# hasindu2008/sigtk

Hardware: AMD Instinct MI355X
Metric: event_raw_samples_per_sec (higher is better)
Workload: dtype f32+f64; 1 GPU; sigtk event (DNA params) on 10000 synthetic reads x 100000 samples per GPU (BASELINE configs[1]), device-resident; reads_per_gpu=10000, samples_per_read=100000, samples_per_gpu=1000000000, fallback_reads=0, rerun_chunks=0, long_detector_replays=66844, long_detector_replay_indices=87529, split_reads=0, batches_in_flight=1, parallelism=reads sharded across ranks, no collective

## Files before the change

### sigtk_amd/build.py

```python
from __future__ import annotations

import os
import shutil
import subprocess
import sys

PKG = os.path.dirname(os.path.abspath(__file__))
ROOT = os.path.dirname(PKG)
CSRC = os.path.join(PKG, "csrc")
HOST = os.path.join(PKG, "host")
LIB = os.path.join(PKG, "libsigtk_gpu.so")
CLI = os.path.join(PKG, "sigtk-amd")
CLI_ASAN = os.path.join(PKG, "sigtk-amd-asan")

EVENT_SOURCES = ["event_launch.hip", "event_whole.hip", "event_seg.hip", "event_multi.hip", "event_fallback.hip"]
HIP_SOURCES = ["api.hip", "api_stat.hip", *EVENT_SOURCES, "stat_launch.hip", "stat_lane.hip", "stat_wave.hip", "stat_long.hip",
               "misc_kernels.hip", "svb_kernels.hip", "sigtext_kernels.hip", "inflate_kernels.hip", "deflate_kernels.hip", "zstd_kernels.hip", "zrec_kernels.hip", "ent_kernels.hip",
               "qts_kernels.hip", "text_kernels.hip", "slow5_text_kernels.hip", "sref_kernels.hip", "ss_kernels.hip", "job.hip", "shims.hip"]
SOURCE_FLAGS = {"event_whole.hip": ["-fno-slp-vectorize"], "event_multi.hip": ["-fno-slp-vectorize"]}
HIPCC_FLAGS = ["--offload-arch=gfx950", "-O3", "-std=c++17", "-ffp-contract=off",
               "-fhip-fp32-correctly-rounded-divide-sqrt", "-fPIC", "-shared", "-Wall",
               "-Wno-unused-function", "-Wno-bitwise-instead-of-logical", "-Wno-c++20-extensions", "-Wno-pass-failed"]


# ... 36 lines not shown
    if jobs:
        with ThreadPoolExecutor(max_workers=min(len(jobs), max(1, (os.cpu_count() or 2) - 1))) as ex:
            list(ex.map(run, jobs))
    if force or jobs or not _newer(LIB, objs):
        run([cc, "--offload-arch=gfx950", "-shared", "-fPIC", "-o", LIB, *objs])
    return LIB


def build_variant(tag: str, defines, sources=(*EVENT_SOURCES, "api.hip"), verbose: bool = False) -> str:
    build_lib(verbose=verbose)
    vdir = os.path.join(PKG, "_variants")
    os.makedirs(vdir, exist_ok=True)
    cc = hipcc()
    flags = [f for f in HIPCC_FLAGS if f != "-shared"] + list(defines)
    objs = []
    for s_ in HIP_SOURCES:
        base = s_[:-4]
        if s_ in sources:
            obj = os.path.join(vdir, "%s_%s.o" % (base, tag))
            cmd = [cc, *flags, *SOURCE_FLAGS.get(s_, []), "-c", "-o", obj, os.path.join(CSRC, s_)]
            if verbose:
                print(" ".join(cmd), file=sys.stderr)
            subprocess.check_call(cmd)
        else:
            obj = os.path.join(PKG, "build", base + ".o")
        objs.append(obj)
    out = os.path.join(vdir, "libsigtk_gpu_%s.so" % tag)
    subprocess.check_call([cc, "--offload-arch=gfx950", "-shared", "-fPIC", "-o", out, *objs])
    return out


def build_cli(force: bool = False, verbose: bool = False) -> str:
    if not os.path.isdir(HOST):
        return ""
    srcs = sorted(os.path.join(HOST, f) for f in os.listdir(HOST) if f.endswith(".c"))
    if not srcs:
        return ""
    deps = srcs + [os.path.join(HOST, f) for f in os.listdir(HOST) if f.endswith(".h")]
    deps.append(os.path.join(ROOT, "include", "sigtk_gpu.h"))
    deps.append(os.path.join(CSRC, "text_format.h"))
    if not force and _newer(CLI, deps) and _newer(CLI, [LIB]):
        return CLI
    cmd = ["gcc", "-O2", "-std=c99", "-D_GNU_SOURCE", "-Wall", "-I", os.path.join(ROOT, "include"), "-o", CLI, *srcs,
           "-L", PKG, "-lsigtk_gpu", "-Wl,-rpath,$ORIGIN", "-Wl,-rpath,/opt/rocm/lib", "-lz", "-lm", "-lpthread"]
    if verbose:
        print(" ".join(cmd), file=sys.stderr)
    subprocess.check_call(cmd)
    return CLI


def build_cli_asan(force: bool = False, verbose: bool = False) -> str:
    srcs = sorted(os.path.join(HOST, f) for f in os.listdir(HOST) if f.endswith(".c"))
    deps = srcs + [os.path.join(HOST, f) for f in os.listdir(HOST) if f.endswith(".h")]
    deps.append(os.path.join(ROOT, "include", "sigtk_gpu.h"))
    deps.append(os.path.join(CSRC, "text_format.h"))
    if not os.path.exists(LIB):
        build_lib(verbose=verbose)
    if not force and _newer(CLI_ASAN, deps) and _newer(CLI_ASAN, [LIB]):
        return CLI_ASAN
    cmd = ["gcc", "-O1", "-g", "-fno-omit-frame-pointer", "-fsanitize=address,undefined", "-fno-sanitize-recover=undefined",
           "-std=c99", "-D_GNU_SOURCE", "-Wall", "-I", os.path.join(ROOT, "include"), "-o", CLI_ASAN, *srcs,
           "-L", PKG, "-lsigtk_gpu", "-Wl,-rpath,$ORIGIN", "-Wl,-rpath,/opt/rocm/lib", "-lz", "-lm", "-lpthread"]
    if verbose:
        print(" ".join(cmd), file=sys.stderr)
    subprocess.check_call(cmd)
    return CLI_ASAN


def build_tools(force: bool = False, verbose: bool = False) -> None:
    tdir = os.path.join(ROOT, "tools")
    math_h = os.path.join(CSRC, "tstat_math.h")
    numerics = ["-ffp-contract=off", "-fhip-fp32-correctly-rounded-divide-sqrt"]
    for name in ("rsq_check", "valu_rate", "fetch_calib", "sqrt_cert_gpu"):
        src = os.path.join(tdir, name + ".hip")
        exe = os.path.join(tdir, name)
        deps = [src] + ([os.path.join(tdir, "valu_rate_tests.inc")] if name == "valu_rate" else [])
        deps += [math_h] if name == "sqrt_cert_gpu" else []
        if not os.path.exists(src) or (not force and _newer(exe, deps)):
            continue
        cmd = [hipcc(), "--offload-arch=gfx950", "-O2", *(numerics if name == "sqrt_cert_gpu" else []), "-o", exe, src]
        if verbose:
            print(" ".join(cmd), file=sys.stderr)
        subprocess.check_call(cmd)
    src, exe = os.path.join(tdir, "sqrt_check.cpp"), os.path.join(tdir, "sqrt_check")
    if os.path.exists(src) and (force or not _newer(exe, [src, math_h])):
        cmd = ["g++", "-O2", "-std=c++17", "-ffp-contract=off", "-pthread", "-o", exe, src]
        if verbose:
            print(" ".join(cmd), file=sys.stderr)
        subprocess.check_call(cmd)


if __name__ == "__main__":
    if "--variant" in sys.argv:
        i = sys.argv.index("--variant")
        print(build_variant(sys.argv[i + 1], [x for x in sys.argv[i + 2:] if x.startswith("-D")], verbose=True))
        sys.exit(0)
    build_tools(force="--force" in sys.argv, verbose=True)
    build_lib(force="--force" in sys.argv, verbose=True)
    build_cli(force="--force" in sys.argv, verbose=True)
    if "--asan" in sys.argv:
        build_cli_asan(force="--force" in sys.argv, verbose=True)
```

### sigtk_amd/csrc/event_detect.h

```cpp
#pragma once
#include <utility>

#include "event_device.h"

namespace sgk {

template <int W1>
struct LzCfg {
    static constexpr int W2 = 2 * W1;
    static constexpr int R = 16;
    static constexpr int NP = (W1 == 3) ? 8 : 16;
    static constexpr int NA = (W1 == 3) ? 4 : 8;
    static constexpr int NL = (W1 == 3) ? 8 : 16;
    static constexpr int H1 = W1 / 2;
};
static_assert(LzCfg<3>::NP >= 8 && LzCfg<7>::NP >= 16, "prefix ring holds P(i) .. P(i+W2+1)");

constexpr int LZ_NONE = -(1 << 29);
constexpr int LZ_NREC = 8;
constexpr int LZ_RING_WORDS = 16;

struct LzSnap {
    LzSnapState init[64];
    LzSnapState at_e[64];
    LzSnapState st0[64];
};
__device__ inline bool lz_equal(const LzSnapState &a, const LzSnapState &b) {
    return a.sp == b.sp && __float_as_int(a.sv) == __float_as_int(b.sv) && a.lm == b.lm && a.r0 == b.r0 &&
           a.bits == b.bits;
}
struct LzLds {
    uint32_t ring[64][LZ_RING_WORDS + 1];
    LzSnap snap;
    LzRun runs[64][LZ_NREC];
    int nrec[64];
};

template <typename T>
__device__ __attribute__((noinline)) float tstat_exact_at(const T *base, Scale sc, int i, int w) {
    double A = 0.0, A2 = 0.0, B = 0.0, B2 = 0.0;
    for (int k = 0; k < w; ++k) {
        const float xa = to_pa(base[i - w + k], sc);
        const float xb = to_pa(base[i + k], sc);
        A = A + (double)xa;
        A2 = A2 + (double)(xa * xa);
        B = B + (double)xb;
        B2 = B2 + (double)(xb * xb);
    }
    if (w == 3) return sgk_tstat_ref<3>(A, A2, B, B2);
    if (w == 6) return sgk_tstat_ref<6>(A, A2, B, B2);
    if (w == 7) return sgk_tstat_ref<7>(A, A2, B, B2);
    return sgk_tstat_ref<14>(A, A2, B, B2);
}

template <typename T>
struct Lead16;
template <>
struct Lead16<int16_t> {
    uint32_t w[8];
    template <int U>
    __device__ __forceinline__ float get(const Scale &sc) const {
        const int v = (U & 1) ? ((int)w[U / 2] >> 16) : (int)(short)(w[U / 2] & 0xffffu);
        const float shifted = (float)v + sc.offf;
        return shifted * sc.unit;
    }
};
template <>
struct Lead16<float> {
    float w[16];
    template <int U>
    __device__ __forceinline__ float get(const Scale &) const { return w[U]; }
};
typedef uint32_t sgk_u32x4_a4 __attribute__((ext_vector_type(4), aligned(4)));

template <typename T>
__device__ __attribute__((noinline)) Lead16<T> lead_fix_head(Lead16<T> g, int pos, T first) {
    T tmp[16];
    __builtin_memcpy(tmp, g.w, sizeof(tmp));
#pragma unroll
    for (int k = 0; k < 16; ++k) tmp[k] = (pos + k < 0) ? first : tmp[k];
    __builtin_memcpy(g.w, tmp, sizeof(tmp));
    return g;
}

constexpr int REP_MAX_EVENTS = 32;
struct RepairCtx {
    const double *P, *P2;
    const int *ev;
    int nev;
    bool all_dirty;
};

__device__ __attribute__((noinline)) float tstat_prefix_at(const double *P, const double *P2, int i, int w) {
    const double p0 = P[i], q0 = P2[i];
    const double A = p0 - P[i - w], A2 = q0 - P2[i - w], B = P[i + w] - p0, B2 = P2[i + w] - q0;
    if (w == 3) return sgk_tstat_ref<3>(A, A2, B, B2);
    if (w == 6) return sgk_tstat_ref<6>(A, A2, B, B2);
    if (w == 7) return sgk_tstat_ref<7>(A, A2, B, B2);
    return sgk_tstat_ref<14>(A, A2, B, B2);
}

template <int W1>
__device__ __forceinline__ void repair_mark(const RepairCtx &rep, int &next_t, int q0, unsigned cnt1, unsigned cnt2,
                                            unsigned &bad1, unsigned &bad2) {
    constexpr int W2 = 2 * W1;
    if (rep.all_dirty) {
#pragma unroll
        for (int u = 0; u < 4; ++u) {
            if ((unsigned)(q0 + u - W1) < cnt1) bad1 |= 1u << u;
            if ((unsigned)(q0 + u - W2) < cnt2) bad2 |= 1u << u;
        }
        return;
    }
    if (next_t > q0 + 3 + W2 - 1) return;
    int nt = 0x7fffffff;
    for (int k = 0; k < rep.nev; ++k) {
        const int t = rep.ev[k];
#pragma unroll
        for (int u = 0; u < 4; ++u) {
            const int i = q0 + u;
            if ((unsigned)(i - t + W1 - 1) < (unsigned)(2 * W1) && (unsigned)(i - W1) < cnt1) bad1 |= 1u << u;
            if ((unsigned)(i - t + W2 - 1) < (unsigned)(2 * W2) && (unsigned)(i - W2) < cnt2) bad2 |= 1u << u;
        }
        if (t + W2 >= q0 + 4 && t < nt) nt = t;
    }
    next_t = nt;
}

constexpr int LZ_PRE = LZ_RING_WORDS;
__device__ __attribute__((noinline)) void lz_emit_slow(uint32_t *ring, unsigned long long *bm, int flushed,
                                                       int i_begin, int s, int e, int p, int cur) {
    const int own_lo = s - i_begin;
    if (p < own_lo) {
        if (cur >= own_lo) ring[LZ_PRE] = (uint32_t)(i_begin + p);
        return;
    }
    if (p >= flushed) {
        atomicOr(&ring[(p >> 5) & (LZ_RING_WORDS - 1)], 1u << (p & 31));
    } else {
        const int pa = i_begin + p;
        if (pa >= s && pa < e) atomicOr(reinterpret_cast<uint32_t *>(bm) + (pa >> 5), 1u << (pa & 31));
    }
}
__device__ __attribute__((noinline)) int lz_record(LzRun *runs, int nrec, int a, int b, int s, int e, int n) {
    if ((b >= s && b < e) || (b == n && e == n && s < n)) {
        if (nrec < LZ_NREC) {
            runs[nrec].a = a;
            runs[nrec].b = b;
        }
        ++nrec;
    }
    return nrec;
}

struct Redo4 {
    float v[4];
};
template <int W1, typename T, bool FLAGGED>
__device__ __attribute__((noinline)) Redo4 redo_quad(const T *base, Scale sc, const double *P, const double *P2, int i0,
                                                     unsigned cnt1, unsigned bits, float t0, float t1, float t2,
                                                     float t3) {
    Redo4 r;
    r.v[0] = t0; r.v[1] = t1; r.v[2] = t2; r.v[3] = t3;
#pragma unroll
    for (int k = 0; k < 4; ++k) {
        if ((bits >> k) & 1u) {
            const int i = i0 + k;
            float v = 0.0f;
            if ((unsigned)(i - W1) < cnt1) {
                if constexpr (FLAGGED) v = tstat_prefix_at(P, P2, i, W1);
                else v = tstat_exact_at<T>(base, sc, i, W1);
            }
            r.v[k] = v;
        }
    }
    return r;
}

typedef unsigned long long lmask_t;
__device__ __forceinline__ bool lane_of(lmask_t m) { return __builtin_amdgcn_inverse_ballot_w64(m); }

template <int W1, typename T, bool FLAGGED>
struct LazyPass {
    using C = LzCfg<W1>;
    static constexpr int W2 = C::W2, R = C::R, NP = C::NP, NA = C::NA, NL = C::NL, H1 = C::H1;
    double Ps[NP], Pq[NP];
    SgkARole ar[NA];
    SgkLSide ls[NL];
    float t1[4];
    lmask_t nk[4];
    lmask_t hc[4];
    Lead16<T> cur;
    float sv;
    int sp;
    lmask_t inpk, val, strong;
    lmask_t hist[H1 + 1];
    uint32_t bw;
    int lm, r0;
    lmask_t hot;
    int nrec;
    uint32_t *ring;
    LzRun *runs;
    const T *base;
    int lo, hi;
    Scale sc;
    int n, s, e, i_begin, ib, jb, flushed;
    unsigned cnt1, cnt2;
    lmask_t done;
    bool slow;
    bool oldpeak;
    unsigned long long *bm;
    RepairCtx rep;
    int next_t;
    int dirty;

    __device__ __forceinline__ void load_lead(Lead16<T> &dst, int pos) const {
        int p = pos > hi - 16 ? hi - 16 : pos;
        p = p < lo ? lo : p;
        constexpr int NV = 16 * (int)sizeof(T) / 16;
        const sgk_u32x4_a4 *src = reinterpret_cast<const sgk_u32x4_a4 *>(base + p);
        sgk_u32x4_a4 v[NV];
#pragma unroll
        for (int k = 0; k < NV; ++k) v[k] = src[k];
        __builtin_memcpy(dst.w, v, sizeof(dst.w));
        if (pos < 0) dst = lead_fix_head<T>(dst, pos, base[0]);
    }

    template <int U>
    __device__ __forceinline__ void tstep() {
        const float xn = cur.template get<U>(sc);
        const float xqn = xn * xn;
        Ps[(U + W2 + 1) % NP] = Ps[(U + W2) % NP] + (double)xn;
        Pq[(U + W2 + 1) % NP] = Pq[(U + W2) % NP] + (double)xqn;
        const double p0 = Ps[U % NP], q0 = Pq[U % NP];
        const double b1 = Ps[(U + W1) % NP] - p0, b1q = Pq[(U + W1) % NP] - q0;
        const double b2 = Ps[(U + W2) % NP] - p0, b2q = Pq[(U + W2) % NP] - q0;
        const SgkLSide lb = sgk_lside<W2>(b2, b2q);
        if constexpr (!FLAGGED) {
            bool cv_ok, tail_ok;
            t1[U & 3] = sgk_tstat_try_ab<W1>(b1, b1q, ar[(U + NA - W1) % NA], cv_ok, tail_ok);
            nk[U & 3] = ~(__ballot(cv_ok) & __ballot(tail_ok));
            ar[U % NA] = sgk_arole<W1, true>(b1, b1q);
            hc[U & 3] = ~__ballot(sgk_long_cold<W2>(ls[(U + NL - W2) % NL], lb));
            ls[U % NL] = lb;
        } else {
            bool ok;
            const float v = sgk_tstat_try_ab<W1>(b1, b1q, ar[(U + NA - W1) % NA], ok);
            ok = ok && sgk_try_domain<W1>(b1, b1q, ar[(U + NA - W1) % NA]);
            const double a_s = Ps[(U + W2) % NP], b_s = (double)xn, r_s = Ps[(U + W2 + 1) % NP];
            const double a_q = Pq[(U + W2) % NP], b_q = (double)xqn, r_q = Pq[(U + W2 + 1) % NP];
            const double t_s = r_s - a_s, t_q = r_q - a_q;
            const double e_s = (a_s - (r_s - t_s)) + (b_s - t_s), e_q = (a_q - (r_q - t_q)) + (b_q - t_q);
            const bool clean = U > dirty;
            if (e_s != 0.0 || e_q != 0.0) dirty = dirty > U + 2 * W2 ? dirty : U + 2 * W2;
            ok = ok && clean;
            ar[U % NA] = sgk_arole<W1, false>(b1, b1q);
            bool cold = sgk_long_cold<W2>(ls[(U + NL - W2) % NL], lb);
            cold = cold && clean && sgk_lside_domain(ls[(U + NL - W2) % NL]) && sgk_lside_domain(lb);
            ls[U % NL] = lb;
            t1[U & 3] = v;
            nk[U & 3] = ~__ballot(ok);
            hc[U & 3] = ~__ballot(cold);
        }
    }

    template <bool SLOW>
    __device__ __forceinline__ void dstep_core(const int u, const float v, const lmask_t hck, const lmask_t live) {
        constexpr float ph = DetParam<W1>::ph, thr1 = DetParam<W1>::thr1;
        const float d1 = v - sv;
        const float ee = lane_of(inpk) ? d1 : -d1;
        lmask_t P = __ballot(ee > 0.0f);
        lmask_t Q = __ballot(ee < -ph);
        const lmask_t Tt = __ballot(v > thr1);
        if constexpr (SLOW) {
            P &= live;
            Q &= live;
        }
        const lmask_t ent = Q & ~inpk;
        const lmask_t pos = (inpk & P) | ent;
        strong = (pos & Tt) | (strong & ~pos);
        lmask_t dom = inpk & strong;
        if constexpr (SLOW) dom &= live;
        val = inpk & (val | (Q & strong));
        lmask_t recent = hist[0];
#pragma unroll
        for (int k = 1; k < H1; ++k) recent |= hist[k];
        lmask_t em = val & ~P & ~recent;
        if constexpr (SLOW) em &= live;
        const lmask_t upd = P | ent | em;
        const uint32_t bit = 1u << ((jb + u - H1 - 1) & 31);
        if (SLOW && oldpeak) {
            if (lane_of(em)) {
                lz_emit_slow(ring, bm, flushed, i_begin, s, e, jb + sp, jb + u);
                lm = sp;
                r0 = u;
            }
        } else {
            if (lane_of(em)) {
                bw |= bit;
                lm = sp;
                r0 = u;
            }
            const lmask_t erare = em & ~hist[H1];
            if (erare != 0ull) {
                if (lane_of(erare)) {
                    bw &= ~bit;
                    const int p = jb + sp, own = s - i_begin;
                    if (p >= own) atomicOr(&ring[(p >> 5) & (LZ_RING_WORDS - 1)], 1u << (p & 31));
                    else if (jb >= own) ring[LZ_PRE] = (uint32_t)(i_begin + p);
                }
            }
        }
        sv = lane_of(upd) ? v : sv;
        sp = lane_of(pos) ? u : sp;
        inpk = (inpk & ~em) | ent;
        val = val & ~em;
// ... 30 lines not shown
    __device__ __forceinline__ void dstep_edge() {
        if constexpr (U == H1 + 1) {
            if ((jb & 16) == 0) bw_advance();
        }
        const lmask_t live = ~done & __ballot((unsigned)(ib + U) < (unsigned)n);
        dstep_core<true>(U, t1[U & 3], hc[U & 3], live);
    }
    __device__ __forceinline__ void slow_fix(const int u0) {
#pragma unroll
        for (int k = 0; k < 4; ++k) {
            const bool in1 = (unsigned)(ib + u0 + k - W1) < cnt1;
            t1[k] = in1 ? t1[k] : 0.0f;
            nk[k] &= __ballot(in1);
            hc[k] &= __ballot((unsigned)(ib + u0 + k - W2) < cnt2);
        }
    }

    template <int U0>
    __device__ __forceinline__ void quad() {
        tstep<U0>();
        tstep<U0 + 1>();
        tstep<U0 + 2>();
        tstep<U0 + 3>();
        if (slow) slow_fix(U0);
        if constexpr (FLAGGED) {
            unsigned bad1 = 0u, bad2 = 0u;
            repair_mark<W1>(rep, next_t, ib + U0, cnt1, cnt2, bad1, bad2);
#pragma unroll
            for (int k = 0; k < 4; ++k) {
                nk[k] |= __ballot(((bad1 >> k) & 1u) != 0u);
                hc[k] |= __ballot(((bad2 >> k) & 1u) != 0u);
            }
        }
        const lmask_t anybad = (nk[0] | nk[1] | nk[2] | nk[3]) & ~done;
        if (anybad != 0ull) {
            if (lane_of(anybad)) {
                const unsigned bits = (lane_of(nk[0]) ? 1u : 0u) | (lane_of(nk[1]) ? 2u : 0u) |
                                      (lane_of(nk[2]) ? 4u : 0u) | (lane_of(nk[3]) ? 8u : 0u);
                const Redo4 r4 = redo_quad<W1, T, FLAGGED>(base, sc, rep.P, rep.P2, ib + U0, cnt1, bits, t1[0], t1[1],
                                                           t1[2], t1[3]);
                t1[0] = r4.v[0]; t1[1] = r4.v[1]; t1[2] = r4.v[2]; t1[3] = r4.v[3];
            }
        }
        if (slow) {
            dstep_edge<U0>();
            dstep_edge<U0 + 1>();
            dstep_edge<U0 + 2>();
            dstep_edge<U0 + 3>();
        } else {
            dstep<U0>();
            dstep<U0 + 1>();
            dstep<U0 + 2>();
            dstep<U0 + 3>();
        }
    }

    template <int K>
    __device__ __forceinline__ void init_step(double &ps, double &pq, const float (&w)[2 * W2], double (&hs)[W2 + 1],
                                              double (&hq)[W2 + 1]) {
        const float x = w[K];
        ps = ps + (double)x;
        pq = pq + (double)(x * x);
        constexpr int k1 = K + 1;
        if constexpr (k1 <= W2) { hs[k1] = ps; hq[k1] = pq; }
        if constexpr (k1 >= W2) { Ps[(k1 - W2) % NP] = ps; Pq[(k1 - W2) % NP] = pq; }
        if constexpr (k1 >= W2 && k1 < W2 + W1) {
            constexpr int pr = k1 - W1;
            ar[((k1 - W1 - W2) % NA + NA) % NA] = sgk_arole<W1, !FLAGGED>(ps - hs[pr], pq - hq[pr]);
        }
        if constexpr (k1 >= W2 && k1 < 2 * W2) {
            constexpr int pr = k1 - W2;
            ls[((k1 - 2 * W2) % NL + NL) % NL] = sgk_lside<W2>(ps - hs[pr], pq - hq[pr]);
        }
    }
    template <int... Ks>
    __device__ __forceinline__ void init_rings(const float (&w)[2 * W2], std::integer_sequence<int, Ks...>) {
        double ps = 0.0, pq = 0.0;
        double hs[W2 + 1], hq[W2 + 1];
        hs[0] = 0.0;
        hq[0] = 0.0;
        (init_step<Ks>(ps, pq, w, hs, hq), ...);
    }

    template <int... Qs>
    __device__ __forceinline__ void block(std::integer_sequence<int, Qs...>) {
        (quad<4 * Qs>(), ...);
    }
};

__device__ __forceinline__ void lz_flush(uint32_t *ring, unsigned long long *bm, int i_begin, int p0, int own_lo,
                                         int own_hi) {
    uint16_t *bm16 = reinterpret_cast<uint16_t *>(bm);
#pragma unroll
    for (int k = 0; k < 8; ++k) {
        const int p = p0 + 32 * k;
        const int wi = (p >> 5) & (LZ_RING_WORDS - 1);
        const uint32_t w = ring[wi];
        ring[wi] = 0u;
        if (p >= own_lo && p < own_hi) bm16[(i_begin + p) >> 4] = (uint16_t)(w & 0xffffu);
        if (p + 16 >= own_lo && p + 16 < own_hi) bm16[(i_begin + p + 16) >> 4] = (uint16_t)(w >> 16);
    }
}

template <int W1, typename T, bool FLAGGED>
__device__ __forceinline__ void pass_lazy(const ReadCtx<T> &rc, bool given, int lead, int steps, bool active, int s,
                                          int e, LzLds *L, const RepairCtx *rep, bool by_progress = false) {
    using LP = LazyPass<W1, T, FLAGGED>;
    constexpr int W2 = LP::W2, R = LP::R;
    if (!__any(active)) return;
    const int l = lane_id();
    LP f;
    f.n = (int)rc.n;
    f.s = active ? s : 0x7fffffff;
    f.e = active ? e : 0x7fffffff;
    f.bm = rc.bm;
    f.sc = rc.sc;
    f.base = rc.base;
    f.lo = (int)(rc.lo < -(1 << 30) ? -(1 << 30) : rc.lo);
    f.hi = (int)(rc.hi > 0x7fffffffLL ? 0x7fffffffLL : rc.hi);
    f.ring = L->ring[l];
    f.runs = L->runs[l];
    const int n = f.n;
    const int i_begin = s - lead;
    f.i_begin = i_begin;
#pragma unroll
    for (int k = 0; k < LZ_RING_WORDS; ++k) f.ring[k] = 0u;
    if (active) f.ring[LZ_PRE] = 0xffffffffu;
#pragma unroll
    for (int k = 0; k < 4; ++k) { f.t1[k] = 0.0f; f.nk[k] = 0ull; f.hc[k] = 0ull; }
    {
        float w[2 * W2];
#pragma unroll
        for (int k = 0; k < 2 * W2; ++k) {
            int p = i_begin - W2 + k;
            p = p > f.hi - 1 ? f.hi - 1 : p;
            p = p < 0 ? 0 : p;
            w[k] = to_pa(f.base[p], f.sc);
        }
#pragma unroll
        for (int k = 0; k < LP::NP; ++k) { f.Ps[k] = 0.0; f.Pq[k] = 0.0; }
        f.init_rings(w, std::make_integer_sequence<int, 2 * W2>{});
        if (i_begin == 0) {
#pragma unroll
            for (int k = 0; k < LP::NA; ++k) f.ar[k].va = __builtin_nan("");
        }
    }
    f.load_lead(f.cur, i_begin + W2);

    f.sv = FLT_MAX;
    f.sp = 0;
    f.inpk = 0ull; f.val = 0ull; f.strong = 0ull; f.hot = 0ull;
#pragma unroll
    for (int k = 0; k <= LP::H1; ++k) f.hist[k] = 0ull;
    f.bw = 0u;
    f.lm = LZ_NONE;
    f.r0 = 0;
    if (__any(given)) {
        LzSnapState st = L->snap.st0[l];
        if (!given) { st.sp = -1; st.sv = FLT_MAX; st.lm = LZ_NONE; st.r0 = i_begin; st.bits = 0u; }
        f.sv = st.sv;
        f.inpk = __ballot((st.bits & 1u) != 0u);
        f.val = __ballot((st.bits & 2u) != 0u);
        f.strong = __ballot((st.bits & 4u) != 0u);
        f.hot = __ballot((st.bits & 8u) != 0u);
        f.sp = (st.bits & 1u) ? st.sp - i_begin : 0;
        f.lm = st.lm == LZ_NONE ? LZ_NONE : st.lm - W1 - i_begin;
#pragma unroll
        for (int k = 0; k <= LP::H1; ++k) f.hist[k] = __ballot((st.bits & 1u) && st.sp == i_begin - 1 - k);
        f.r0 = st.r0 - i_begin;
    }
    f.nrec = 0;
    f.done = ~__ballot(active);
    f.flushed = 0;
    if constexpr (FLAGGED) {
        f.dirty = 2 * W2;
        f.rep = *rep;
        f.next_t = 0x7fffffff;
        for (int k = 0; k < f.rep.nev; ++k) {
            const int t = f.rep.ev[k];
            if (t + W2 >= i_begin && t < f.next_t) f.next_t = t;
        }
    }
    const int main_steps = steps;
    f.cnt1 = (n - 2 * W1 + 1) > 0 ? (unsigned)(n - 2 * W1 + 1) : 0u;
    f.cnt2 = (n - 2 * W2 + 1) > 0 ? (unsigned)(n - 2 * W2 + 1) : 0u;
    const int own_lo = lead, own_hi = active ? lead + (e - s) : lead;

    auto snapshot = [&](int ib) -> LzSnapState {
        LzSnapState st;
        const bool ip = lane_of(f.inpk);
        st.sv = f.sv;
        st.sp = ip ? ib + f.sp : -1;
        st.lm = (f.lm + W1 < 0) ? LZ_NONE : ib + f.lm + W1;
        st.r0 = ib + max(f.r0, f.lm + W1 + 1);
        st.bits = (ip ? 1u : 0u) | ((ip && lane_of(f.val)) ? 2u : 0u) | ((ip && lane_of(f.strong)) ? 4u : 0u) |
                  (lane_of(f.hot) ? 8u : 0u);
        return st;
    };

    constexpr int PRIO_STEPS = 400;
    const int q1 = by_progress ? main_steps - 3 * PRIO_STEPS : -1, q2 = by_progress ? main_steps - 2 * PRIO_STEPS : -1,
              q3 = by_progress ? main_steps - PRIO_STEPS : -1;
    if (by_progress) {
        if (q1 > 0) __builtin_amdgcn_s_setprio(3);
        else if (q2 > 0) __builtin_amdgcn_s_setprio(2);
        else if (q3 > 0) __builtin_amdgcn_s_setprio(1);
        else __builtin_amdgcn_s_setprio(0);
    }
    int jb = 0;
    for (;;) {
        const int ib = i_begin + jb;
        if ((jb & 255) == 0 && jb >= 512) {
            lz_flush(f.ring, f.bm, i_begin, jb - 512, own_lo, own_hi);
            f.flushed = jb - 256;
        }
        const bool lane_edge = ib + R - 1 > n - W2;
        const lmask_t old_peak = __ballot(f.sp < -(256 - 2 * R)) | (__ballot(f.sp + jb < own_lo) & __ballot(jb == own_lo));
        f.oldpeak = (old_peak & f.inpk & ~f.done) != 0ull;
        f.slow = f.oldpeak || (__ballot(lane_edge) & ~f.done) != 0ull;
        f.ib = ib;
        f.jb = jb;
        Lead16<T> nxt;
        f.load_lead(nxt, ib + R + W2);
        f.block(std::make_integer_sequence<int, R / 4>{});
        f.cur = nxt;
        f.sp -= R;
        f.lm = f.lm < LZ_NONE ? LZ_NONE : f.lm - R;
// ... 6 lines not shown
        {
            const int nb = i_begin + jb;
            if (active && lead > 0 && jb == lead) L->snap.init[l] = snapshot(nb);
            if (active && nb == e) L->snap.at_e[l] = snapshot(nb);
            const lmask_t reach = __ballot(nb >= e) & ~f.done;
            if ((reach & f.hot) != 0ull) {
                if (lane_of(reach & f.hot) && e == n) f.nrec = lz_record(f.runs, f.nrec, nb + max(f.r0, f.lm + W1 + 1), n, s, e, n);
            }
            f.done |= reach;
            f.inpk &= ~reach;
            f.val &= ~reach;
            f.strong &= ~reach;
        }
        if (jb >= main_steps && f.done == ~0ull) break;
    }
    {
        const int p = jb - LP::H1 - 2 < 0 ? 0 : jb - LP::H1 - 2;
        atomicOr(&f.ring[(p >> 5) & (LZ_RING_WORDS - 1)], f.bw);
    }
    for (int p0 = f.flushed; p0 < jb; p0 += 256) lz_flush(f.ring, f.bm, i_begin, p0, own_lo, own_hi);
    if (active) L->nrec[l] = f.nrec;
}

template <int W1, typename T, bool FLAGGED, bool COLLECT = false>
__device__ inline void replay_run(const ReadCtx<T> &rc, const RepairCtx *rep, bool has, int i, int b, int bits_lo,
                           int bits_hi, EvHeader *hdr, int *found = nullptr) {
    if (has && b > i) atomicAdd(&hdr->n_replay_idx, (unsigned long long)(b - i));
    constexpr int W2 = 2 * W1;
    constexpr float ph = DetParam<W1>::ph, thr2 = DetParam<W1>::thr2;
    const int n = (int)rc.n;
    const unsigned cnt2 = (n - 2 * W2 + 1) > 0 ? (unsigned)(n - 2 * W2 + 1) : 0u;
    uint32_t *bm32 = reinterpret_cast<uint32_t *>(rc.bm);
    int lp = -1;
    float lv = FLT_MAX;
    bool lvalid = false;
    while (__any(has && i < b)) {
        if (has && i < b) {
            float v2 = 0.0f;
            if ((unsigned)(i - W2) < cnt2) {
                if constexpr (FLAGGED) v2 = tstat_prefix_at(rep->P, rep->P2, i, W2);
                else v2 = tstat_exact_at<T>(rc.base, rc.sc, i, W2);
            }
            if (lp < 0) {
                if (v2 < lv) {
                    lv = v2;
                } else if (v2 - lv > ph) {
                    lv = v2;
                    lp = i;
                }
            } else {
                if (v2 > lv) {
                    lv = v2;
                    lp = i;
                }
                if (lv - v2 > ph && lv > thr2) lvalid = true;
                if (lvalid && (i - lp) > W2 / 2) {
                    if (lp > 0 && lp < n && lp >= bits_lo && lp < bits_hi) {
                        if constexpr (COLLECT) *found = 1;
                        else atomicOr(&bm32[lp >> 5], 1u << (lp & 31));
                    }
                    lp = -1;
                    lv = v2;
                    lvalid = false;
                }
            }
            ++i;
        }
    }
}
template <int W1, typename T, bool FLAGGED>
__device__ void replay_long_runs(const ReadCtx<T> &rc, LzLds *L, const RepairCtx *rep, bool active, int bits_lo,
                                 EvHeader *hdr) {
    const int l = lane_id();
    const int nrec = active ? L->nrec[l] : 0;
    for (int k = 0; k < LZ_NREC; ++k) {
        const bool has = k < nrec;
        if (!__any(has)) break;
        const int i = has ? L->runs[l][k].a : 0;
        const int b = has ? L->runs[l][k].b : 0;
        replay_run<W1, T, FLAGGED>(rc, rep, has, i, b, bits_lo, 0x7fffffff, hdr);
    }
}

template <int W1, typename T, bool FLAGGED, bool MULTI = false>
__device__ __forceinline__ int detect_span(const ReadCtx<T> &rc, EvHeader *hdr, LzLds *L, const RepairCtx *rep,
                                           const int a, const int b, const int mode, const int lead_override,
                                           SegState *seg, const int lanes = 64) {
    const int n = (int)rc.n;
    if constexpr (!MULTI) {
        if (b <= a) return 0;
    }
    const int len = b - a;
    int lead = len < 32768 ? LEAD_DNA_SHORT : LEAD_DNA;
    if (W1 == 7) lead = len <= 32768 ? LEAD_RNA_SHORT : LEAD_RNA;
    if constexpr (MULTI) {
        const long long len64 = (long long)len * (64 / lanes);
        lead = len64 < 32768 ? LEAD_DNA_SHORT : LEAD_DNA;
        if (W1 == 7) lead = len64 <= 32768 ? LEAD_RNA_SHORT : LEAD_RNA;
    }
    if (lead_override > 0) lead = lead_override;
    const bool no_fast = (reinterpret_cast<uintptr_t>(rc.base) & 3u) != 0 || rc.hi < (int64_t)n + 16;
    if constexpr (!MULTI) {
        if (no_fast) return 1;
    }
    const int c = MULTI ? (lane_id() & (lanes - 1)) : lane_id();
    int K, s, e0, lead_c;
    if (mode == 1) {
        K = 16 * ((len + 1023) / 1024);
        s = a + c * K;
        e0 = s + K;
        lead_c = lead;
    } else {
        K = MULTI ? chunk_len_lanes(len, lead, lanes) : chunk_len_fast(len, lead);
        s = c == 0 ? a : a + c * K + lead;
        e0 = c == 0 ? a + lead + K : s + K;
        lead_c = c > 0 ? lead : 0;
    }
    int TT = lead + K;
    int Kmax = K;
    if constexpr (MULTI) {
#pragma unroll
        for (int d = 32; d >= 1; d >>= 1) {
            const int o = __shfl_xor(Kmax, d, 64), t = __shfl_xor(TT, d, 64);
            Kmax = o > Kmax ? o : Kmax;
            TT = t > TT ? t : TT;
        }
    }
    const int e = e0 < b ? e0 : b;
    const bool active = s < b && !(MULTI && no_fast);
    {
        LzSnapState z;
        z.sp = -1; z.sv = FLT_MAX; z.lm = LZ_NONE; z.r0 = 0; z.bits = 0u;
        L->snap.init[lane_id()] = z;
        L->snap.at_e[lane_id()] = z;
        L->nrec[lane_id()] = 0;
        L->ring[lane_id()][LZ_PRE] = 0xffffffffu;
    }
    bool run = active;
    bool first = true;
    const int l = lane_id();
    const uint32_t pol = FLAGGED ? 0u : prio_policy(rc.dev);
    for (int iter = 0; iter < 66; ++iter) {
        pass_lazy<W1, T, FLAGGED>(rc, first ? (mode == 2 && c == 0) : true, first ? lead_c : 0, first ? TT : Kmax, run, s, e,
                                  L, rep, first && (pol == 1u || pol == 2u));
        __syncthreads();
        const LzSnapState pe = L->snap.at_e[c > 0 ? l - 1 : l];
        const LzSnapState mine = L->snap.init[l];
        const bool bad = active && c > 0 && !lz_equal(pe, mine);
        const unsigned long long badmask = __ballot(bad);
        if (badmask == 0ull) break;
        __syncthreads();
        if (bad) {
            L->snap.init[l] = pe;
            L->snap.st0[l] = pe;
        }
        run = bad;
        first = false;
        if (l == 0) atomicAdd(&hdr->n_rerun, (uint32_t)__popcll(badmask));
        __syncthreads();
    }
    int rcode = 0;
    if constexpr (MULTI) {
        const unsigned long long over = __ballot(active && L->nrec[l] > LZ_NREC);
        const unsigned long long grp = (lanes >= 64 ? ~0ull : ((1ull << lanes) - 1ull)) << (l & ~(lanes - 1));
        if (no_fast) rcode = 1;
        else if (over & grp) rcode = 2;
    } else {
        if (__any(active && L->nrec[l] > LZ_NREC)) return 2;
    }
    const bool mine_ok = active && rcode == 0;
    if (seg) {
        const int last = __popcll(__ballot(active)) - 1;
        if (l == 0) {
            seg->init0 = L->snap.init[0];
            seg->end = L->snap.at_e[last];
        }
        const int nrec = active ? L->nrec[l] : 0;
        int ncross = 0;
        for (int k = 0; k < nrec; ++k) ncross += (L->runs[l][k].a < a) ? 1 : 0;
        const int incl = wave_incl_scan_i(ncross);
        const int total = wave_last_i(incl);
        if (total > SEG_CROSS_MAX) rcode = 2;
        else {
            int at = incl - ncross;
            for (int k = 0; k < nrec; ++k) {
                if (L->runs[l][k].a < a) seg->cross[at++] = L->runs[l][k];
            }
        }
        if (l == 0) seg->n_cross = total > SEG_CROSS_MAX ? 0u : (uint32_t)total;
    }
    const int pre = mine_ok ? (int)L->ring[l][LZ_PRE] : -1;
    const bool pre_out = pre >= 0 && pre < a;
    if (seg) {
        const int npre = pre_out ? 1 : 0;
        const int incl = wave_incl_scan_i(npre);
        const int total = wave_last_i(incl);
        if (total > SEG_PRE_MAX) rcode = 2;
        else if (npre) seg->pre[incl - 1] = pre;
        if (l == 0) seg->n_pre = total > SEG_PRE_MAX ? 0u : (uint32_t)total;
    }
    const unsigned long long hotm = __ballot(mine_ok && L->nrec[l] > 0);
    const bool anypre = __any(pre >= 0);
    if (hotm != 0ull || anypre) {
        if (l == 0 && hotm != 0ull) atomicAdd(&hdr->n_hot_runs, (uint32_t)__popcll(hotm));
        __threadfence_block();
        __syncthreads();
        if (pre >= 0 && !pre_out) atomicOr(reinterpret_cast<uint32_t *>(rc.bm) + (pre >> 5), 1u << (pre & 31));
        if (hotm != 0ull) replay_long_runs<W1, T, FLAGGED>(rc, L, rep, mine_ok, a, hdr);
    }
    return rcode;
}
template <int W1, typename T, bool FLAGGED>
__device__ __forceinline__ int detect_read_lazy(const ReadCtx<T> &rc, EvHeader *hdr, LzLds *L, const RepairCtx *rep) {
    const int n = (int)rc.n;
    if (n <= 0) return 0;
    return detect_span<W1, T, FLAGGED>(rc, hdr, L, rep, 0, n, 0, 0, nullptr);
}

}
```

### sigtk_amd/csrc/event_multi.hip

```cpp
#include "event_build.h"

namespace sgk {

template <int W1, typename T>
__global__ __launch_bounds__(64, (W1 == 3 ? DET_WAVES_DNA : DET_WAVES_RNA)) void k_event_multi(EvArgs a) {
    __shared__ EventLds L;
    const int lanes = (int)a.multi_lanes, G = 64 / lanes;
    const int l = lane_id();
    const uint32_t first = a.order ? a.order[a.n_reads + len_bucket(a.multi_max)] : 0u;
    const uint32_t nshort = a.n_reads - first;
    const uint32_t w0 = blockIdx.x * (uint32_t)G;
    if (w0 >= nshort) return;
    const uint32_t gi = (uint32_t)l / (uint32_t)lanes;
    const bool has = w0 + gi < nshort;
    const uint32_t idx = first + (has ? w0 + gi : w0);
    const uint32_t r = a.order ? a.order[idx] : idx;
    ReadCtx<T> rc = make_ctx<T>(a, r);
    const bool mine = has && !(a.max_segs && rc.n >= (int64_t)a.long_min);
    if (!mine) rc.n = 0;
    const int rcode = detect_span<W1, T, false, true>(rc, a.hdr, &L.lz, nullptr, 0, (int)rc.n, 0, a.lead_override, nullptr,
                                                      lanes);
    __builtin_amdgcn_fence(__ATOMIC_RELEASE, "workgroup");
    __syncthreads();
    __builtin_amdgcn_fence(__ATOMIC_ACQUIRE, "workgroup");
    for (int g = 0; g < G; ++g) {
        if (w0 + (uint32_t)g >= nshort) break;
        const uint32_t rg = (uint32_t)__builtin_amdgcn_readlane((int)r, g * lanes);
        const int code = __builtin_amdgcn_readlane(rcode, g * lanes);
        if (!__builtin_amdgcn_readlane((int)mine, g * lanes)) continue;
        const ReadCtx<T> rcg = make_ctx<T>(a, rg);
        build_read<T>(a, rcg, rg, &L.b, code != 0);
        __syncthreads();
    }
}

int launch_k_event_multi(int rna, bool float_input, hipStream_t st, const EvArgs &a) {
    const uint32_t per_wave = 64u / a.multi_lanes;
    const uint32_t grid = (a.n_reads + per_wave - 1) / per_wave;
    if (rna && float_input) SGK_LAUNCH("k_event_multi", (k_event_multi<7, float>), grid, 64, st, a);
    else if (rna) SGK_LAUNCH("k_event_multi", (k_event_multi<7, int16_t>), grid, 64, st, a);
    else if (float_input) SGK_LAUNCH("k_event_multi", (k_event_multi<3, float>), grid, 64, st, a);
    else SGK_LAUNCH("k_event_multi", (k_event_multi<3, int16_t>), grid, 64, st, a);
    return SGK_OK;
}

}
```

### sigtk_amd/csrc/event_whole.hip

```cpp
#include "event_build.h"

namespace sgk {

template <int W1, typename T>
__global__ __launch_bounds__(64, (W1 == 3 ? DET_WAVES_DNA : DET_WAVES_RNA)) void k_event(EvArgs a) {
    __shared__ EventLds L;
    const uint32_t bi = blockIdx.x;
    const uint32_t r = a.order ? a.order[bi] : bi;
    const ReadCtx<T> rc = make_ctx<T>(a, r);
    if (seg_len_of(a, bi, (uint32_t)rc.n) != 0u) return;
    if (a.multi_lanes && rc.n < (int64_t)a.multi_max) return;
#ifdef SGK_DEV
    unsigned long long t0 = 0ull, t1 = 0ull;
    if (a.dev & SGK_DEV_TRACE) t0 = wall_clock64();
    int rcode = 0;
    if (!(a.dev & SGK_DEV_NO_DETECT)) rcode = detect_span<W1, T, false>(rc, a.hdr, &L.lz, nullptr, 0, (int)rc.n, 0, a.lead_override, nullptr);
    if (a.dev & SGK_DEV_TRACE) t1 = wall_clock64();
#else
    const int rcode = detect_span<W1, T, false>(rc, a.hdr, &L.lz, nullptr, 0, (int)rc.n, 0, a.lead_override, nullptr);
#endif
    __builtin_amdgcn_fence(__ATOMIC_RELEASE, "workgroup");
    __syncthreads();
    __builtin_amdgcn_fence(__ATOMIC_ACQUIRE, "workgroup");
#ifdef SGK_DEV
    if (!(a.dev & SGK_DEV_NO_BUILD)) build_read<T>(a, rc, r, &L.b, rcode != 0);
    if ((a.dev & SGK_DEV_TRACE) && lane_id() == 0) {
        unsigned hw, xcc;
        asm volatile("s_getreg_b32 %0, hwreg(HW_REG_HW_ID)" : "=s"(hw));
        asm volatile("s_getreg_b32 %0, hwreg(HW_REG_XCC_ID)" : "=s"(xcc));
        unsigned long long *tr = reinterpret_cast<unsigned long long *>(a.scratch) + 4ull * blockIdx.x;
        tr[0] = t0;
        tr[1] = t1;
        tr[2] = wall_clock64();
        tr[3] = ((unsigned long long)xcc << 32) | hw;
    }
#else
    build_read<T>(a, rc, r, &L.b, rcode != 0);
#endif
}

int launch_k_event(int rna, bool float_input, hipStream_t st, const EvArgs &a) {
    if (rna && float_input) SGK_LAUNCH("k_event", (k_event<7, float>), a.n_reads, 64, st, a);
    else if (rna) SGK_LAUNCH("k_event", (k_event<7, int16_t>), a.n_reads, 64, st, a);
    else if (float_input) SGK_LAUNCH("k_event", (k_event<3, float>), a.n_reads, 64, st, a);
    else SGK_LAUNCH("k_event", (k_event<3, int16_t>), a.n_reads, 64, st, a);
    return SGK_OK;
}

}
```

### sigtk_amd/csrc/tstat_math.h

```cpp
#pragma once
#include <math.h>
#include <stdint.h>
#include <string.h>

#if defined(__HIPCC__)
#define SGK_TM __host__ __device__ inline
#define SGK_TM_COLD __host__ __device__ __attribute__((noinline))
#else
#define SGK_TM static inline
#define SGK_TM_COLD static __attribute__((noinline))
#endif

#ifndef SGK_RSQ64
#if defined(__HIP_DEVICE_COMPILE__)
#define SGK_RSQ64(v) __builtin_amdgcn_rsq(v)
#else
#define SGK_RSQ64(v) (1.0 / sqrt(v))
#endif
#endif

SGK_TM uint64_t sgk_d2u(double x) {
    uint64_t u;
    memcpy(&u, &x, 8);
    return u;
// ... 84 lines not shown
        const f2 q = a * r;
        const f2 rem = __builtin_elementwise_fma(-q, d, a);
        return __builtin_elementwise_fma(rem, r, q);
    };
    const f2 sum2 = {(float)B1, (float)B2};
    const f2 sumsq2 = {(float)B1q, (float)B2q};
    const f2 mean1 = {(float)sgk_div_f64<W>(A1), (float)sgk_div_f64<2 * W>(A2)};
    const f2 mean2 = div2(sum2);
    const f2 m1sq = mean1 * mean1;
    const f2 m2sq = mean2 * mean2;
    const f2 q2 = div2(sumsq2);
    double acc1 = sgk_div_f64<W>(A1q);
    double acc2 = sgk_div_f64<2 * W>(A2q);
    acc1 = acc1 - (double)m1sq.x;
    acc2 = acc2 - (double)m1sq.y;
    acc1 = acc1 + (double)q2.x;
    acc2 = acc2 + (double)q2.y;
    acc1 = acc1 - (double)m2sq.x;
    acc2 = acc2 - (double)m2sq.y;
    f2 cv = {fmaxf((float)acc1, FMIN), fmaxf((float)acc2, FMIN)};
    const f2 delta = mean2 - mean1;
    const f2 cvd = div2(cv);
    const bool fl1 = cv.x == FMIN, fl2 = cv.y == FMIN;
    const float cvw1 = fl1 ? FMIN / (float)W : cvd.x;
    const float cvw2 = fl2 ? FMIN / (float)(2 * W) : cvd.y;
    bool t1ok, t2ok;
    v1 = sgk_tail_fast(delta.x, cvw1, t1ok);
    v2 = sgk_tail_fast(delta.y, cvw2, t2ok);
    ok1 = (fminf(fminf(fabsf(sum2.x), sumsq2.x), fl1 ? 1.0f : cv.x) >= SGK_F32_TINY) & t1ok;
    ok2 = (fminf(fminf(fabsf(sum2.y), sumsq2.y), fl2 ? 1.0f : cv.y) >= SGK_F32_TINY) & t2ok;
#else
    v1 = sgk_tstat_try<W>(A1, A1q, B1, B1q, ok1);
    v2 = sgk_tstat_try<2 * W>(A2, A2q, B2, B2q, ok2);
#endif
}


#ifndef SGK_RSQ32
#if defined(__HIP_DEVICE_COMPILE__)
#define SGK_RSQ32(v) __builtin_amdgcn_rsqf(v)
#else
#define SGK_RSQ32(v) ((float)(1.0 / sqrt((double)(v))))
#endif
#endif

SGK_TM float sgk_tail_f32(float delta, float cvw, bool &ok) {
    const float ad = fabsf(delta);
    const float y0 = SGK_RSQ32(cvw);
    const float s0 = cvw * y0;
    const float e = fmaf(-s0, s0, cvw);
    const float yh = 0.5f * y0;
    const float sl = e * yh;
    const float q0 = ad * y0;
    const float r1 = fmaf(-q0, s0, ad);
    const float rho = fmaf(-q0, sl, r1);
    const float ql = rho * y0;
    const float m = q0 * 1.8189894035458565e-12f;
    const float lo = q0 + (ql - m);
    const float hi = q0 + (ql + m);
    ok = lo == hi;
    return lo;
}

struct SgkARole {
    float mean1;
    double va;
};
template <int W, bool SHORT = false>
SGK_TM SgkARole sgk_arole(double S, double Sq) {
    SgkARole a;
    if (SHORT) {
        constexpr double r = 1.0 / (double)W;
        a.mean1 = (float)(S * r);
    } else {
        a.mean1 = (float)sgk_div_f64<W>(S);
    }
    const float m1sq = a.mean1 * a.mean1;
    a.va = sgk_div_f64<W>(Sq) - (double)m1sq;
    return a;
}
#define SGK_CV_MIN 8.0779356694631609e-28f

template <int W>
SGK_TM float sgk_tstat_try_ab(double S, double Sq, const SgkARole &a, bool &cv_ok, bool &tail_ok) {
    const float sum2 = (float)S;
    const float sumsq2 = (float)Sq;
    const float mean2 = sgk_div_f32<W>(sum2);
    const float m2sq = mean2 * mean2;
    const float q2 = sgk_div_f32<W>(sumsq2);
    double acc = a.va + (double)q2;
    acc = acc - (double)m2sq;
    const float cv = (float)acc;
    cv_ok = cv > SGK_CV_MIN;
    const float delta = mean2 - a.mean1;
    const float cvw = sgk_div_f32<W>(cv);
    return sgk_tail_f32(delta, cvw, tail_ok);
}
template <int W>
SGK_TM float sgk_tstat_try_ab(double S, double Sq, const SgkARole &a, bool &ok) {
    bool cv_ok, tail_ok;
    const float v = sgk_tstat_try_ab<W>(S, Sq, a, cv_ok, tail_ok);
    ok = cv_ok & tail_ok;
    return v;
}

SGK_TM uint32_t sgk_f2u(float x) {
    uint32_t u;
    memcpy(&u, &x, 4);
    return u;
}
SGK_TM bool sgk_band60(float x) {
    const uint32_t e = (sgk_f2u(x) >> 23) & 0xffu;
    return x == 0.0f || (e - 67u) < 120u;
}
template <int W>
SGK_TM bool sgk_try_domain(double S, double Sq, const SgkARole &a) {
    const float sum2 = (float)S;
    const float sumsq2 = (float)Sq;
    const float mean2 = sgk_div_f32<W>(sum2);
    const float m2sq = mean2 * mean2;
    const float q2 = sgk_div_f32<W>(sumsq2);
    double acc = a.va + (double)q2;
    acc = acc - (double)m2sq;
    const float cv = (float)acc;
    const float delta = mean2 - a.mean1;
    const uint32_t ed = (sgk_f2u(delta) >> 23) & 0xffu;
    const bool d_ok = delta == 0.0f || (ed - 67u) < 100u;
    return sgk_band60(sum2) & sgk_band60(sumsq2) & d_ok & (cv < 1152921504606846976.0f);
}

#ifndef SGK_RCP32
#if defined(__HIP_DEVICE_COMPILE__)
#define SGK_RCP32(v) __builtin_amdgcn_rcpf(v)
#else
#define SGK_RCP32(v) (1.0f / (v))
#endif
#endif
SGK_TM float sgk_refined_rcp(float b) {
    const float r0 = SGK_RCP32(b);
    const float e = fmaf(-b, r0, 1.0f);
    return fmaf(e, r0, r0);
}
SGK_TM float sgk_div_with_rcp(float a, float b, float r1) {
    const float q0 = a * r1;
    const float rem0 = fmaf(-b, q0, a);
    const float q1 = fmaf(rem0, r1, q0);
    const float rem1 = fmaf(-b, q1, a);
    return fmaf(rem1, r1, q1);
}

#define SGK_SQRT_LO 0x1F800000u
#define SGK_SQRT_HI 0x54000000u
SGK_TM float sgk_sqrt_cert(float v, bool &dom_ok, bool &cert_ok) {
    dom_ok = (sgk_f2u(v) - SGK_SQRT_LO) < (SGK_SQRT_HI - SGK_SQRT_LO);
    const float y0 = SGK_RSQ32(v);
    const float s0 = v * y0;
    const float e = fmaf(-s0, s0, v);
    const float yh = 0.5f * y0;
    const float sl = e * yh;
    const float lo = s0 + fmaf(s0, -9.094947017729282e-13f, sl);
    const float hi = s0 + fmaf(s0, 9.094947017729282e-13f, sl);
    cert_ok = lo == hi;
    return lo;
}
SGK_TM float sgk_sqrt_cert(float v, bool &ok) {
    bool dom_ok, cert_ok;
    const float s = sgk_sqrt_cert(v, dom_ok, cert_ok);
    ok = dom_ok & cert_ok;
    return s;
}

struct SgkLSide {
    float m, q, v;
};
template <int W>
SGK_TM SgkLSide sgk_lside(double S, double Sq) {
    SgkLSide s;
    s.m = (float)S;
    s.q = (float)Sq * (float)W;
    s.v = fmaf(-s.m, s.m, s.q);
    return s;
}
SGK_TM bool sgk_lside_domain(const SgkLSide &s) {
    return sgk_band60(s.q) & sgk_band60(s.m);
}
template <int W>
SGK_TM bool sgk_long_cold(const SgkLSide &a, const SgkLSide &b) {
    const float V = a.v + b.v;
    const float Qs = a.q + b.q;
    const float rhs = fmaf(Qs, -81.0f * 1.9073486328125e-06f, 81.0f * V);
    const float D = b.m - a.m;
    const float Ms = fabsf(a.m) + fabsf(b.m);
    const float Dub = fmaf(Ms, 9.5367431640625e-07f, fabsf(D));
    const float lhs = (Dub * Dub) * ((float)W * (1.0f + 1.52587890625e-05f));
    return lhs < rhs;
}

template <int W>
SGK_TM float sgk_tstat_fast(double A, double A2, double B, double B2) {
    bool ok;
    const float tq = sgk_tstat_try<W>(A, A2, B, B2, ok);
    if (ok) return tq;
    __asm__ volatile("" ::: "memory");
    return sgk_tstat_ref<W>(A, A2, B, B2);
}

template <int W>
SGK_TM_COLD float sgk_tstat_ref(double A, double A2, double B, double B2) {
    const float wf = (float)W;
    const float sum2 = (float)B;
    const float sumsq2 = (float)B2;
    const float mean1 = (float)(A / (double)wf);
    const float mean2 = sum2 / wf;
    const float m1sq = mean1 * mean1;
    const float m2sq = mean2 * mean2;
    const float q2 = sumsq2 / wf;
    double acc = A2 / (double)wf;
    acc = acc - (double)m1sq;
    acc = acc + (double)q2;
    acc = acc - (double)m2sq;
    float cv = (float)acc;
    cv = fmaxf(cv, 1.17549435e-38f);
    const float delta = mean2 - mean1;
    const float cvw = cv / wf;
    return (float)(fabs((double)delta) / sqrt((double)cvw));
}
```

Before: 299.1 billion samples/s.

## Add lead-path lazy pass reusing short-window sums for long-window stats

Adds a LEAD variant of the lazy detection pass that keeps rings of float short-window sums and reuses them. The long-window side statistics are built from two adjacent short halves instead of separate f64 prefix differences, and the per-step arole/tstat work is restructured around those rings. It is enabled by default for the DNA whole-read kernel through SGK_EVENT_LEAD=1, while the multi-read kernel stays opt-in. This is meant to cut the f64 subtraction and conversion work per step. In exchange it uses more registers for larger rings and changes rounding, since the long side now sums two f32 halves; a new host check tool is added to the build, apparently to validate this.

```diff
diff --git a/sigtk_amd/build.py b/sigtk_amd/build.py
--- a/sigtk_amd/build.py
+++ b/sigtk_amd/build.py
@@ -142,12 +142,13 @@
         if verbose:
             print(" ".join(cmd), file=sys.stderr)
         subprocess.check_call(cmd)
-    src, exe = os.path.join(tdir, "sqrt_check.cpp"), os.path.join(tdir, "sqrt_check")
-    if os.path.exists(src) and (force or not _newer(exe, [src, math_h])):
-        cmd = ["g++", "-O2", "-std=c++17", "-ffp-contract=off", "-pthread", "-o", exe, src]
-        if verbose:
-            print(" ".join(cmd), file=sys.stderr)
-        subprocess.check_call(cmd)
+    for name in ("sqrt_check", "long_cold_check"):
+        src, exe = os.path.join(tdir, name + ".cpp"), os.path.join(tdir, name)
+        if os.path.exists(src) and (force or not _newer(exe, [src, math_h])):
+            cmd = ["g++", "-O2", "-std=c++17", "-ffp-contract=off", "-pthread", "-o", exe, src]
+            if verbose:
+                print(" ".join(cmd), file=sys.stderr)
+            subprocess.check_call(cmd)
 
 
 if __name__ == "__main__":
diff --git a/sigtk_amd/csrc/event_detect.h b/sigtk_amd/csrc/event_detect.h
--- a/sigtk_amd/csrc/event_detect.h
+++ b/sigtk_amd/csrc/event_detect.h
@@ -16,6 +16,10 @@
 };
 static_assert(LzCfg<3>::NP >= 8 && LzCfg<7>::NP >= 16, "prefix ring holds P(i) .. P(i+W2+1)");
 
+#ifndef SGK_EVENT_LEAD
+#define SGK_EVENT_LEAD 1
+#endif
+
 constexpr int LZ_NONE = -(1 << 29);
 constexpr int LZ_NREC = 8;
 constexpr int LZ_RING_WORDS = 16;
@@ -180,12 +184,17 @@
 typedef unsigned long long lmask_t;
 __device__ __forceinline__ bool lane_of(lmask_t m) { return __builtin_amdgcn_inverse_ballot_w64(m); }
 
-template <int W1, typename T, bool FLAGGED>
+template <int W1, typename T, bool FLAGGED, bool LEAD = false>
 struct LazyPass {
+    static_assert(!(LEAD && FLAGGED), "the fallback keeps its domain checks and TwoSum form");
     using C = LzCfg<W1>;
     static constexpr int W2 = C::W2, R = C::R, NP = C::NP, NA = C::NA, NL = C::NL, H1 = C::H1;
+    static constexpr int NA2 = LEAD ? 2 * NA : NA;
+    static constexpr int NS = LEAD ? NA : 1;
+    static_assert(NA2 > (LEAD ? 2 : 1) * W1 && (!LEAD || NS > W1) && R % NA2 == 0, "ring depths");
     double Ps[NP], Pq[NP];
-    SgkARole ar[NA];
+    SgkARole ar[NA2];
+    float ss[NS], sqs[NS];
     SgkLSide ls[NL];
     float t1[4];
     lmask_t nk[4];
@@ -232,6 +241,21 @@
         const float xqn = xn * xn;
         Ps[(U + W2 + 1) % NP] = Ps[(U + W2) % NP] + (double)xn;
         Pq[(U + W2 + 1) % NP] = Pq[(U + W2) % NP] + (double)xqn;
+        if constexpr (LEAD) {
+            const double c = Ps[(U + W2) % NP] - Ps[(U + W1) % NP], cq = Pq[(U + W2) % NP] - Pq[(U + W1) % NP];
+            const float s_p = (float)c, sq_p = (float)cq;
+            const float s_i = ss[U % NS], sq_i = sqs[U % NS];
+            ss[(U + W1) % NS] = s_p;
+            sqs[(U + W1) % NS] = sq_p;
+            bool cv_ok, tail_ok;
+            t1[U & 3] = sgk_tstat_try_ab<W1>(s_i, sq_i, ar[(U + NA2 - W1) % NA2], cv_ok, tail_ok);
+            nk[U & 3] = ~(__ballot(cv_ok) & __ballot(tail_ok));
+            ar[(U + W1) % NA2] = sgk_arole<W1, true>(c, cq);
+            const SgkLSide lb = sgk_lside_halves<W2>(s_i, sq_i, s_p, sq_p);
+            hc[U & 3] = ~__ballot(sgk_long_cold<W2>(ls[(U + NL - W2) % NL], lb));
+            ls[U % NL] = lb;
+            return;
+        }
         const double p0 = Ps[U % NP], q0 = Pq[U % NP];
         const double b1 = Ps[(U + W1) % NP] - p0, b1q = Pq[(U + W1) % NP] - q0;
         const double b2 = Ps[(U + W2) % NP] - p0, b2q = Pq[(U + W2) % NP] - q0;
@@ -428,6 +452,30 @@
         (init_step<Ks>(ps, pq, w, hs, hq), ...);
     }
 
+    __device__ __forceinline__ void init_lead(const float (&w)[2 * W2]) {
+        double hs[2 * W2 + 1], hq[2 * W2 + 1];
+        hs[0] = 0.0;
+        hq[0] = 0.0;
+#pragma unroll
+        for (int k = 0; k < 2 * W2; ++k) {
+            hs[k + 1] = hs[k] + (double)w[k];
+            hq[k + 1] = hq[k] + (double)(w[k] * w[k]);
+        }
+#pragma unroll
+        for (int k = W2; k <= 2 * W2; ++k) { Ps[(k - W2) % NP] = hs[k]; Pq[(k - W2) % NP] = hq[k]; }
+        float sf[W2 + W1], sqf[W2 + W1];
+#pragma unroll
+        for (int j = 0; j < W2 + W1; ++j) {
+            const double c = hs[j + W1] - hs[j], cq = hq[j + W1] - hq[j];
+            sf[j] = (float)c;
+            sqf[j] = (float)cq;
+            if (j >= W1) ar[(j - W2 + NA2) % NA2] = sgk_arole<W1, true>(c, cq);
+            if (j >= W2) { ss[(j - W2) % NS] = sf[j]; sqs[(j - W2) % NS] = sqf[j]; }
+        }
+#pragma unroll
+        for (int j = 0; j < W2; ++j) ls[(j - W2 + NL) % NL] = sgk_lside_halves<W2>(sf[j], sqf[j], sf[j + W1], sqf[j + W1]);
+    }
+
     template <int... Qs>
     __device__ __forceinline__ void block(std::integer_sequence<int, Qs...>) {
         (quad<4 * Qs>(), ...);
@@ -448,10 +496,10 @@
     }
 }
 
-template <int W1, typename T, bool FLAGGED>
+template <int W1, typename T, bool FLAGGED, bool LEAD = false>
 __device__ __forceinline__ void pass_lazy(const ReadCtx<T> &rc, bool given, int lead, int steps, bool active, int s,
                                           int e, LzLds *L, const RepairCtx *rep, bool by_progress = false) {
-    using LP = LazyPass<W1, T, FLAGGED>;
+    using LP = LazyPass<W1, T, FLAGGED, LEAD>;
     constexpr int W2 = LP::W2, R = LP::R;
     if (!__any(active)) return;
     const int l = lane_id();
@@ -485,10 +533,16 @@
         }
 #pragma unroll
         for (int k = 0; k < LP::NP; ++k) { f.Ps[k] = 0.0; f.Pq[k] = 0.0; }
-        f.init_rings(w, std::make_integer_sequence<int, 2 * W2>{});
+        if constexpr (LEAD) f.init_lead(w);
+        else f.init_rings(w, std::make_integer_sequence<int, 2 * W2>{});
         if (i_begin == 0) {
-#pragma unroll
-            for (int k = 0; k < LP::NA; ++k) f.ar[k].va = __builtin_nan("");
+            if constexpr (LEAD) {
+#pragma unroll
+                for (int k = 1; k <= W1; ++k) f.ar[LP::NA2 - k].va = __builtin_nan("");
+            } else {
+#pragma unroll
+                for (int k = 0; k < LP::NA; ++k) f.ar[k].va = __builtin_nan("");
+            }
         }
     }
     f.load_lead(f.cur, i_begin + W2);
@@ -661,7 +715,7 @@
     }
 }
 
-template <int W1, typename T, bool FLAGGED, bool MULTI = false>
+template <int W1, typename T, bool FLAGGED, bool MULTI = false, bool LEAD = false>
 __device__ __forceinline__ int detect_span(const ReadCtx<T> &rc, EvHeader *hdr, LzLds *L, const RepairCtx *rep,
                                            const int a, const int b, const int mode, const int lead_override,
                                            SegState *seg, const int lanes = 64) {
@@ -720,8 +774,8 @@
     const int l = lane_id();
     const uint32_t pol = FLAGGED ? 0u : prio_policy(rc.dev);
     for (int iter = 0; iter < 66; ++iter) {
-        pass_lazy<W1, T, FLAGGED>(rc, first ? (mode == 2 && c == 0) : true, first ? lead_c : 0, first ? TT : Kmax, run, s, e,
-                                  L, rep, first && (pol == 1u || pol == 2u));
+        pass_lazy<W1, T, FLAGGED, LEAD>(rc, first ? (mode == 2 && c == 0) : true, first ? lead_c : 0, first ? TT : Kmax, run,
+                                        s, e, L, rep, first && (pol == 1u || pol == 2u));
         __syncthreads();
         const LzSnapState pe = L->snap.at_e[c > 0 ? l - 1 : l];
         const LzSnapState mine = L->snap.init[l];
diff --git a/sigtk_amd/csrc/event_multi.hip b/sigtk_amd/csrc/event_multi.hip
--- a/sigtk_amd/csrc/event_multi.hip
+++ b/sigtk_amd/csrc/event_multi.hip
@@ -18,8 +18,9 @@
     ReadCtx<T> rc = make_ctx<T>(a, r);
     const bool mine = has && !(a.max_segs && rc.n >= (int64_t)a.long_min);
     if (!mine) rc.n = 0;
-    const int rcode = detect_span<W1, T, false, true>(rc, a.hdr, &L.lz, nullptr, 0, (int)rc.n, 0, a.lead_override, nullptr,
-                                                      lanes);
+    constexpr bool MULTI_LEAD = W1 == 3 && ((SGK_EVENT_LEAD) & 4) != 0;
+    const int rcode = detect_span<W1, T, false, true, MULTI_LEAD>(rc, a.hdr, &L.lz, nullptr, 0, (int)rc.n, 0,
+                                                                  a.lead_override, nullptr, lanes);
     __builtin_amdgcn_fence(__ATOMIC_RELEASE, "workgroup");
     __syncthreads();
     __builtin_amdgcn_fence(__ATOMIC_ACQUIRE, "workgroup");
diff --git a/sigtk_amd/csrc/event_whole.hip b/sigtk_amd/csrc/event_whole.hip
--- a/sigtk_amd/csrc/event_whole.hip
+++ b/sigtk_amd/csrc/event_whole.hip
@@ -1,6 +1,9 @@
 #include "event_build.h"
 
 namespace sgk {
+
+template <int W1>
+constexpr bool EV_LEAD = ((SGK_EVENT_LEAD) & (W1 == 3 ? 1 : 2)) != 0;
 
 template <int W1, typename T>
 __global__ __launch_bounds__(64, (W1 == 3 ? DET_WAVES_DNA : DET_WAVES_RNA)) void k_event(EvArgs a) {
@@ -14,10 +17,10 @@
     unsigned long long t0 = 0ull, t1 = 0ull;
     if (a.dev & SGK_DEV_TRACE) t0 = wall_clock64();
     int rcode = 0;
-    if (!(a.dev & SGK_DEV_NO_DETECT)) rcode = detect_span<W1, T, false>(rc, a.hdr, &L.lz, nullptr, 0, (int)rc.n, 0, a.lead_override, nullptr);
+    if (!(a.dev & SGK_DEV_NO_DETECT)) rcode = detect_span<W1, T, false, false, EV_LEAD<W1>>(rc, a.hdr, &L.lz, nullptr, 0, (int)rc.n, 0, a.lead_override, nullptr);
     if (a.dev & SGK_DEV_TRACE) t1 = wall_clock64();
 #else
-    const int rcode = detect_span<W1, T, false>(rc, a.hdr, &L.lz, nullptr, 0, (int)rc.n, 0, a.lead_override, nullptr);
+    const int rcode = detect_span<W1, T, false, false, EV_LEAD<W1>>(rc, a.hdr, &L.lz, nullptr, 0, (int)rc.n, 0, a.lead_override, nullptr);
 #endif
     __builtin_amdgcn_fence(__ATOMIC_RELEASE, "workgroup");
     __syncthreads();
diff --git a/sigtk_amd/csrc/tstat_math.h b/sigtk_amd/csrc/tstat_math.h
--- a/sigtk_amd/csrc/tstat_math.h
+++ b/sigtk_amd/csrc/tstat_math.h
@@ -190,9 +190,7 @@
 #define SGK_CV_MIN 8.0779356694631609e-28f
 
 template <int W>
-SGK_TM float sgk_tstat_try_ab(double S, double Sq, const SgkARole &a, bool &cv_ok, bool &tail_ok) {
-    const float sum2 = (float)S;
-    const float sumsq2 = (float)Sq;
+SGK_TM float sgk_tstat_try_ab(float sum2, float sumsq2, const SgkARole &a, bool &cv_ok, bool &tail_ok) {
     const float mean2 = sgk_div_f32<W>(sum2);
     const float m2sq = mean2 * mean2;
     const float q2 = sgk_div_f32<W>(sumsq2);
@@ -203,6 +201,10 @@
     const float delta = mean2 - a.mean1;
     const float cvw = sgk_div_f32<W>(cv);
     return sgk_tail_f32(delta, cvw, tail_ok);
+}
+template <int W>
+SGK_TM float sgk_tstat_try_ab(double S, double Sq, const SgkARole &a, bool &cv_ok, bool &tail_ok) {
+    return sgk_tstat_try_ab<W>((float)S, (float)Sq, a, cv_ok, tail_ok);
 }
 template <int W>
 SGK_TM float sgk_tstat_try_ab(double S, double Sq, const SgkARole &a, bool &ok) {
@@ -286,6 +288,14 @@
     SgkLSide s;
     s.m = (float)S;
     s.q = (float)Sq * (float)W;
+    s.v = fmaf(-s.m, s.m, s.q);
+    return s;
+}
+template <int W>
+SGK_TM SgkLSide sgk_lside_halves(float s1, float sq1, float s2, float sq2) {
+    SgkLSide s;
+    s.m = s1 + s2;
+    s.q = (sq1 + sq2) * (float)W;
     s.v = fmaf(-s.m, s.m, s.q);
     return s;
 }
```

After: 304.8 billion samples/s, median of 6. 1.9% higher.
